# zhaihongjia/SplatLoc

Hardware: AMD Instinct MI355X
Metric: fwd+bwd frames/s @1080p, 500k Gaussians, 32 feat-ch; HBM GB/s vs roofline (higher is better)
Workload: dtype f32

## Files before the change

include/splatraster.h:

```cpp
#ifndef SPLATRASTER_H
#define SPLATRASTER_H

#include <stddef.h>
#include <stdint.h>

#ifdef __cplusplus
extern "C" {
#endif

#define SPLATRASTER_ABI_VERSION 20

#define SPLATRASTER_TILE 16

#define SPLATRASTER_OK 0
#define SPLATRASTER_ERR_BAD_ARG 1
#define SPLATRASTER_ERR_HIP 2
#define SPLATRASTER_ERR_UNSUPPORTED 3
#define SPLATRASTER_ERR_OVERFLOW 4
#define SPLATRASTER_WARN_LOOKBACK_STALL 5

typedef struct splatraster_settings {
    int32_t image_height;
    int32_t image_width;
    float tanfovx;
// ... 557 lines not shown
                               float* grad_h, uint8_t* valid, void* stream);

#define SPLATRASTER_GRAD_MASK_REPLICA 0
#define SPLATRASTER_GRAD_MASK_GLOBAL 1
int splatraster_grad_mask_workspace_bytes(int32_t N, int32_t H, int32_t W, int32_t mode, int32_t have_intensity, size_t* bytes);
int splatraster_grad_mask(int32_t N, int32_t H, int32_t W, const float* images, float edge_threshold, float eps, int32_t mode,
                          int32_t out_u8, void* out, float* intensity, float* thresholds, void* workspace, size_t workspace_bytes,
                          void* stream);
int splatraster_debug_image_ops_path(int32_t H, int32_t W);

int splatraster_masked_median_workspace_bytes(int32_t N, int64_t n, size_t* bytes);
int splatraster_masked_median(int32_t N, int64_t n, const float* values, int32_t positive_only, const float* opacity,
                              float opacity_min, const uint8_t* mask, float* median, float* std, int64_t* count, uint8_t* valid,
                              void* workspace, size_t workspace_bytes, void* stream);



int splatraster_sp_nms_tile(int32_t* tile_h, int32_t* tile_w);
int splatraster_sp_workspace_bytes(int32_t B, int32_t H, int32_t W, int32_t max_keypoints, size_t* bytes);
int splatraster_sp_scores(int32_t B, int32_t Hc, int32_t Wc, const float* semi, float* scores, void* stream);
int splatraster_sp_nms(int32_t B, int32_t H, int32_t W, const float* scores, int32_t radius, float* out, void* stream);
int splatraster_sp_select(int32_t B, int32_t H, int32_t W, const float* nms, float threshold, int32_t max_keypoints, int32_t border,
                          float* keypoints, float* scores, int32_t* count, int32_t* candidates, void* workspace, size_t workspace_bytes,
                          void* stream);
int splatraster_sp_sample(int32_t B, int32_t Hc, int32_t Wc, const float* coarse, int32_t K, const float* keypoints, const int32_t* count,
                          float* descriptors, void* workspace, size_t workspace_bytes, void* stream);
int splatraster_sp_dense_descriptors(int32_t B, int32_t Hc, int32_t Wc, const float* coarse, int32_t row0, int32_t rows, float* out,
                                     void* workspace, size_t workspace_bytes, void* stream);


int splatraster_poll_errors(void);
int splatraster_debug_set_spin_limit(uint32_t limit);
int splatraster_debug_set_deterministic(int on);
int splatraster_debug_set_small_panel_max_waves(int waves);
int splatraster_debug_set_split_max_waves(int waves);
int splatraster_debug_set_fwd_team(int mode);
int splatraster_debug_set_payload_stream_min(int64_t instances);
int splatraster_debug_set_payload_compact(int mode);
int splatraster_debug_set_dead_marks(int on);
int splatraster_debug_set_front_end(int mode);
int splatraster_debug_set_tile_sort_cap(int keys);
int splatraster_debug_set_sort_fork(int mode);
int splatraster_debug_exp2(int64_t n, const float* x, float* y, void* stream);
int splatraster_debug_poison_lds(uint32_t pattern, void* stream);

const char* splatraster_error_string(int status);
const char* splatraster_last_hip_error(void);
int splatraster_abi_version(void);

#ifdef __cplusplus
}
#endif
#endif
```

splatloc_amd/_native.py:

```python
from __future__ import annotations

import ctypes as C
import os

from . import build as _build

_LIB = None
ABI_VERSION = 20
ERR_UNSUPPORTED = 3

OK = 0
WARN_LOOKBACK_STALL = 5
_ERR_NAMES = {1: "bad argument", 2: "HIP runtime error", 3: "unsupported configuration",
              4: "tile instance count overflow", 5: "look-back stall (results late, never wrong)"}


class Settings(C.Structure):
    _fields_ = [
        ("image_height", C.c_int32),
        ("image_width", C.c_int32),
        ("tanfovx", C.c_float),
        ("tanfovy", C.c_float),
        ("scale_modifier", C.c_float),
        ("sh_degree", C.c_int32),
# ... 213 lines not shown
    "splatraster_densify_workspace_bytes": (_sz, [_i32]),
    "splatraster_densify_plan": (C.c_int, [C.POINTER(Model), _vp, _vp, C.c_float, C.c_float, C.c_float, C.c_float, _i32,
                                           _i32, _vp, C.POINTER(_i32), _vp]),
    "splatraster_densify_plan_thresholds": (C.c_int, [C.POINTER(Model), _vp, _vp, C.c_float, C.c_float, C.c_float,
                                                      C.c_float, _i32, _i32, _vp, C.POINTER(_i32), _vp]),
    "splatraster_densify_apply": (C.c_int, [C.POINTER(Model), C.POINTER(Model), C.POINTER(Model), _vp, C.c_uint64,
                                            C.c_uint64, _vp, _i32, C.POINTER(Model), C.POINTER(Model), C.POINTER(Model),
                                            _vp, _vp, _vp]),
    "splatraster_model_append": (C.c_int, [C.POINTER(Model)] * 7 + [_vp]),
    "splatraster_adam_step": (C.c_int, [_i32, C.POINTER(AdamGroup), C.c_double, C.c_double, C.c_double, C.c_float, _vp]),
    "splatraster_adam_step_radii": (C.c_int, [_i32, C.POINTER(AdamGroup), C.c_double, C.c_double, C.c_double, C.c_float, _i32, _vp, _vp, _vp]),
    "splatraster_adam_step_gated": (C.c_int, [_i32, C.POINTER(AdamGroup), C.c_double, C.c_double, C.c_double, C.c_float, _vp, _vp]),
    "splatraster_adam_step_radii_gated": (C.c_int, [_i32, C.POINTER(AdamGroup), C.c_double, C.c_double, C.c_double, C.c_float, _i32, _vp,
                                                    _vp, _vp, _vp]),
    "splatraster_isotropic_loss_workspace_bytes": (_sz, [_i32]),
    "splatraster_isotropic_loss": (C.c_int, [_i32, _i32, _vp, _vp, _vp, _vp, _vp, _vp]),
    "splatraster_mapping_loss_workspace_bytes": (_sz, [_i32]),
    "splatraster_mapping_loss": (C.c_int, [_i32] + [_vp] * 6 + [C.c_float] + [_vp] * 7),
    "splatraster_mapping_loss_window": (C.c_int, [_i32, _i32, _vp, C.c_float, _vp, _vp, _vp]),
    "splatraster_refinement_loss_workspace_bytes": (_sz, [_i32, _i32, _i32]),
    "splatraster_refinement_loss": (C.c_int, [_i32, _i32, _i32, C.c_float] + [_vp] * 6),
    "splatraster_eval_metrics_workspace_bytes": (_sz, [_i32, _i32, _i32]),
    "splatraster_eval_metrics": (C.c_int, [_i32, _i32, _i32] + [_vp] * 5),
    "splatraster_l1_rgbd_loss": (C.c_int, [_i64, _vp, _vp, _i64, _vp, _vp, C.c_float, _vp, _vp, _vp, _vp]),
    "splatraster_pose_step": (C.c_int, [_vp] * 5 + [C.c_float] * 5 + [C.c_int] + [_vp] * 5),
    "splatraster_l1_rgbd_loss_window": (C.c_int, [_i32, C.POINTER(L1View), _i64, _i64, C.c_float, _vp, _vp]),
    "splatraster_pose_step_window": (C.c_int, [_i32] + [_vp] * 5 + [C.c_float] * 5 + [C.c_int] + [_vp] * 5),
    "splatraster_error_string": (C.c_char_p, [C.c_int]),
    "splatraster_last_hip_error": (C.c_char_p, []),
    "splatraster_abi_version": (C.c_int, []),
    "splatraster_poll_errors": (C.c_int, []),
    "splatraster_debug_set_spin_limit": (C.c_int, [C.c_uint32]),
    "splatraster_debug_set_deterministic": (C.c_int, [C.c_int]),
    "splatraster_debug_exp2": (C.c_int, [_i64, _vp, _vp, _vp]),
    "splatraster_debug_poison_lds": (C.c_int, [C.c_uint32, _vp]),
}


def lib_path() -> str:
    return _build.LIB_PATH


def load(build_if_missing: bool = True):
    global _LIB
    if _LIB is not None:
        return _LIB
    path = os.environ.get("SPLATRASTER_LIB", _build.LIB_PATH)
    if path == _build.LIB_PATH and build_if_missing and _build.have_hipcc():
        try:
            _build.build()
        except Exception as e:
            raise RuntimeError(
                "splatloc_amd: the HIP extension libsplatraster.so could not be built "
                f"({e}). There is no CPU fallback.") from e
    if not os.path.exists(path):
        raise RuntimeError(f"{path} is missing and hipcc is not available: run `python -m splatloc_amd.build` "
                           "on a machine with ROCm. There is no CPU fallback.")
    lib = C.CDLL(path)
    lib.splatraster_abi_version.restype = C.c_int
    got = int(lib.splatraster_abi_version())
    if got != ABI_VERSION:
        raise RuntimeError(f"{path} has ABI version {got}, this binding needs {ABI_VERSION}: stale library, "
                           "rebuild with `python -m splatloc_amd.build --force`")
    for name, (res, args) in SYMBOLS.items():
        fn = getattr(lib, name)
        fn.restype = res
# ... 81 lines not shown
```

splatloc_amd/csrc/capi.hip:

```cpp
#include <assert.h>
#include <string.h>

#include <mutex>
#include <unordered_map>
#include <string>
#include <vector>

#include "common.h"

namespace sr {

static thread_local std::string g_last_error;
static int g_deterministic = 0;
static int g_split_max_waves = SPLIT_MAX_WAVES;
static int g_fwd_team = -1;
static int g_payload_compact = -1;
static int g_dead_marks = 1;
static int g_bin_mode = -1;

void set_hip_error(hipError_t e, const char* what)
{
    g_last_error = std::string(what) + ": " + hipGetErrorString(e);
}

// ... 1000 lines not shown
    return SPLATRASTER_OK;
}

int splatraster_debug_set_split_max_waves(int waves)
{
    g_split_max_waves = waves < 0 ? SPLIT_MAX_WAVES : (waves > SPLIT_MAX_WAVES ? SPLIT_MAX_WAVES : waves);
    return SPLATRASTER_OK;
}

int splatraster_debug_set_fwd_team(int mode)
{
    g_fwd_team = mode < 0 ? -1 : (mode > 2 ? 2 : mode);
    return SPLATRASTER_OK;
}

int splatraster_mark_visible(int32_t P, const float* means3D, const float* viewmatrix,
                             const float* projmatrix, uint8_t* present, void* stream)
{
    (void)projmatrix;
    if (P < 0) return SPLATRASTER_ERR_BAD_ARG;
    if (P == 0) return SPLATRASTER_OK;
    if (!means3D || !viewmatrix || !present) return SPLATRASTER_ERR_BAD_ARG;
    return launch_mark_visible(P, means3D, viewmatrix, present, reinterpret_cast<hipStream_t>(stream));
}

int splatraster_poll_errors(void) { return lookback_error_poll(); }

int splatraster_debug_set_deterministic(int on)
{
    g_deterministic = on ? 1 : 0;
    return SPLATRASTER_OK;
}

int splatraster_debug_set_spin_limit(uint32_t limit)
{
    int st = lookback_error_init();
    if (st) return st;
    return lookback_set_spin_limit(limit);
}

int splatraster_debug_exp2(int64_t n, const float* x, float* y, void* stream)
{
    if (n < 0) return SPLATRASTER_ERR_BAD_ARG;
    if (n == 0) return SPLATRASTER_OK;
    if (!x || !y) return SPLATRASTER_ERR_BAD_ARG;
    return launch_debug_exp2(n, x, y, reinterpret_cast<hipStream_t>(stream));
}

int splatraster_debug_poison_lds(uint32_t pattern, void* stream)
{
    return launch_poison_lds(pattern, reinterpret_cast<hipStream_t>(stream));
}

size_t splatraster_sort_tmp_bytes(int64_t n)
{
    const size_t m = (size_t)(n > 0 ? n : 1);
    return align_up(4 * m, 256) * 2 + sort_tmp_bytes(n);
}

static int sort_in_place(bool keys16, int64_t n, uint32_t* keys, uint32_t* vals, int32_t key_bits, void* tmp, void* stream_)
{
    if (!keys || !vals || !tmp) return SPLATRASTER_ERR_BAD_ARG;
    {
        int st0 = lookback_error_init();
        if (st0) return st0;
    }
// ... 91 lines not shown
```

splatloc_amd/csrc/common.h:

```cpp
#pragma once
#include <hip/hip_runtime.h>
#include <stdint.h>

#include "../../include/splatraster.h"

namespace sr {

constexpr int TILE = SPLATRASTER_TILE;
constexpr int TILE_PIX = TILE * TILE;
constexpr float NEAR_Z = 0.2f;
constexpr float DILATION = 0.3f;
constexpr float ALPHA_MAX = 0.99f;
constexpr float ALPHA_MIN = 1.0f / 255.0f;
constexpr float T_EPS = 0.0001f;
constexpr int WAVE = 64;
constexpr int PREPROCESS_BLOCK = 256;
static inline int preprocess_blocks(int32_t P) { return (P + PREPROCESS_BLOCK - 1) / PREPROCESS_BLOCK; }

void set_hip_error(hipError_t e, const char* what);
void set_error_text(const char* text);

int lookback_error_init();
int lookback_error_poll();
int lookback_set_spin_limit(uint32_t limit);
// ... 207 lines not shown
    uint32_t capacity;
    uint32_t tag;
    uint32_t* status;
    uint32_t* mirror;
};
struct BoundedStatus {
    uint32_t* dev;
    uint32_t* host;
    uint32_t* host_dev;
    int device;
};
int launch_bounded_status_clear(const BoundedStatus& st, hipStream_t stream);
int launch_bin_scatter_sort(const FramePlan& p, const GeomView& g, const uint32_t* table, const BinView& b, uint64_t* keys,
                            hipStream_t stream, const BoundedRun* bd = nullptr);

int launch_emit(const FramePlan& p, int64_t R, const GeomView& g, uint32_t* keys, uint32_t* vals, uint32_t* ranges,
                uint32_t nranges, hipStream_t stream, bool keys16 = false );
int launch_ranges_clear(int32_t tiles, uint32_t* ranges, hipStream_t stream);
int launch_payload(const FramePlan& p, int64_t R, const GeomView& g, const BinView& b, hipStream_t stream);
int launch_payload_compact(const FramePlan& p, int64_t R, const GeomView& g, const BinView& b, uint32_t* cranges, hipStream_t stream);
int launch_pad_features(int32_t P, int C, const float* feat, float* featp, hipStream_t stream);
static inline int padded_channels(int C) { return (C + 3) & ~3; }
constexpr int POSE_SETS = 16, POSE_SET_FLOATS = 64;
constexpr size_t POSE_ACC_BYTES = (size_t)POSE_SETS * POSE_SET_FLOATS * sizeof(float) + 256;
constexpr int POSE_ACC_FLOATS = (int)(POSE_ACC_BYTES / sizeof(float));
__host__ __device__ constexpr int gacc_moment_offset(int C) { return ((C & 15) + 7 <= 16) ? C : ((C + 15) & ~15); }
__host__ __device__ constexpr int gacc_row_floats(int C) { return (gacc_moment_offset(C) + 7 + 15) & ~15; }
__host__ __device__ constexpr int gacc_shared_floats(int C) { return C >= 32 ? (C & ~15) : 0; }
__host__ __device__ constexpr int gacc_view_floats(int C) { return gacc_row_floats(C) - gacc_shared_floats(C); }
__host__ __device__ static inline size_t gacc_total_floats(int C, size_t P, size_t V)
{
    return P * (size_t)gacc_shared_floats(C) + V * P * (size_t)gacc_view_floats(C);
}
struct GaccLayout {
    uint32_t SH, PV;
    uint32_t P;
    __host__ __device__ size_t index(size_t g, size_t i, uint32_t col) const
    {
        return col < SH ? i * SH + col : (size_t)P * SH + g * PV + (col - SH);
    }
    __host__ __device__ uint32_t view_base24(uint32_t row0) const { return P * SH + row0 * PV - SH; }
    __host__ __device__ uint32_t stride24(uint32_t col) const { return col < SH ? SH : PV; }
    __host__ __device__ uint32_t base24(uint32_t col, uint32_t row0) const { return col < SH ? 0u : view_base24(row0); }
};
__host__ __device__ constexpr int gacc_det_headroom_drop(int C, int V) { return (gacc_shared_floats(C) > 0 && V > 1) ? 3 : 0; }
__host__ __device__ static inline GaccLayout gacc_layout(int C, int32_t P)
{
    return GaccLayout{(uint32_t)gacc_shared_floats(C), (uint32_t)gacc_view_floats(C), (uint32_t)P};
}
#ifndef SR_SPLIT_MAX_WAVES
#define SR_SPLIT_MAX_WAVES 6144
#endif
constexpr int SPLIT_MAX_WAVES = SR_SPLIT_MAX_WAVES;
constexpr int SPLIT_MIN_LIST = 256;
#ifndef SR_SPLIT_PARTS
#define SR_SPLIT_PARTS 4
#endif
constexpr int SPLIT_PARTS = SR_SPLIT_PARTS;
constexpr int SPLIT_PARTS_MAX = 4 * SPLIT_PARTS;
#ifndef SR_SPLIT_LONG
#define SR_SPLIT_LONG 1024
#endif
#ifndef SR_SPLIT_EXTRA_TILES
#define SR_SPLIT_EXTRA_TILES 512
#endif
constexpr int SPLIT_LONG = SR_SPLIT_LONG, SPLIT_EXTRA_TILES = SR_SPLIT_EXTRA_TILES;
// ... 31 lines not shown
```

splatloc_amd/csrc/composite_bwd.hip:

```cpp
#include <type_traits>

#include "composite_common.h"

#ifndef SR_BWD_FS
#define SR_BWD_FS 32
#endif
#ifndef SR_BWD_STAGE_UNROLL
#define SR_BWD_STAGE_UNROLL 3
#endif

#ifndef SR_BWD_MINW
#define SR_BWD_MINW 4
#endif

#ifndef SR_BWD_DOT_CHAINS
#define SR_BWD_DOT_CHAINS 2
#endif
#ifndef SR_BWD_SMALL_PANEL_MAX_WAVES
#define SR_BWD_SMALL_PANEL_MAX_WAVES 6144
#endif
#ifndef SR_BWD_DOT_PREFETCH
#define SR_BWD_DOT_PREFETCH 1
#endif
#ifndef SR_BWD_TM
// ... 33 lines not shown
{
    const int eb = (int)((max_bits >> 23) & 0xffu);
    return DET_HEADROOM_EXP - (eb > 0 ? eb : 1);
}
template <bool DET>
__device__ __forceinline__ void acc_add(float* gacc, long long* gacc64, size_t idx, float v, int det_pass, int det_drop)
{
    if (DET) {
        if (det_pass == 0) {
            atomicMax(reinterpret_cast<unsigned*>(gacc) + idx, __float_as_uint(fabsf(v)));
        } else {
            const unsigned mb = __builtin_nontemporal_load(reinterpret_cast<const unsigned*>(gacc) + idx);
            if (((mb >> 23) & 0xffu) == 0xffu) {
                if (__builtin_isinf(v)) atomicAdd(reinterpret_cast<unsigned long long*>(gacc64) + idx, v > 0.f ? 1ull : (1ull << 32));
                return;
            }
            const double scaled = ldexp((double)v, det_scale_exp(mb) - det_drop);
            atomicAdd(reinterpret_cast<unsigned long long*>(gacc64) + idx, (unsigned long long)__double2ll_rn(scaled));
        }
    } else {
        (void)det_pass;
        (void)det_drop;
        atomicAdd(gacc + idx, v);
    }
}

__device__ __forceinline__ float walk_divide(float T, float one_minus_alpha) { return T * __builtin_amdgcn_rcpf(one_minus_alpha); }
__device__ __forceinline__ double walk_divide(double T, double one_minus_alpha) { return T / one_minus_alpha; }
__device__ __forceinline__ float walk_fma(float a, float b, float c) { return fmaf(a, b, c); }
__device__ __forceinline__ double walk_fma(double a, double b, double c) { return fma(a, b, c); }
template <typename ST>
__device__ __forceinline__ void walk_entry(ST& T, ST& A, bool hit, float alpha, float q, float& dA, float& w)
{
    const ST Ti = hit ? walk_divide(T, (ST)1 - (ST)alpha) : T;
    const ST d = (ST)q - A;
    dA = (float)(Ti * d);
    const ST ah = hit ? (ST)alpha : (ST)0;
    A = walk_fma(ah, d, A);
    w = (float)(ah * Ti);
    T = Ti;
}

enum class GaccTable { SHARED, VIEW, BY_COLUMN };
template <bool DET>
struct GradRows {
    float* __restrict__ gacc;
    long long* __restrict__ gacc64;
    GaccLayout GL;
    uint32_t row0, pv_base;
    int det_pass, det_drop;
    __device__ __forceinline__ uint32_t stride(uint32_t col, GaccTable tb) const
    {
        return tb == GaccTable::SHARED ? GL.SH : (tb == GaccTable::VIEW ? GL.PV : GL.stride24(col));
    }
    __device__ __forceinline__ uint32_t offset(uint32_t col, GaccTable tb) const
    {
        return (tb == GaccTable::SHARED ? 0u : (tb == GaccTable::VIEW ? pv_base : GL.base24(col, row0))) + col;
    }
    static __device__ __forceinline__ size_t index(uint32_t id, uint32_t stride, uint32_t offset) { return (size_t)(__umul24(id, stride) + offset); }
    __device__ __forceinline__ size_t index(uint32_t id, uint32_t col, GaccTable tb) const { return index(id, stride(col, tb), offset(col, tb)); }
    __device__ __forceinline__ void add(size_t idx, float v) const { acc_add<DET>(gacc, gacc64, idx, v, det_pass, det_drop); }
};

template <int NC, bool SP, bool AUX>
constexpr int bwd_min_waves() { return (BwdCfg<NC, SP, AUX>::TM && NC >= 32) ? SR_BWD_MINW_TM : SR_BWD_MINW; }

template <int NC, bool DET, bool SP, bool AUX>
__global__ void __launch_bounds__(WAVE, (bwd_min_waves<NC, SP, AUX>()))
composite_bwd_kernel(int W, int H, int C_total, int CP4, int c0, int first_pass, int tiles , int V,
                     int P ,
                     const uint32_t* __restrict__ ranges, const uint32_t* __restrict__ ipack ,
                     const float4* __restrict__ irec, const float4* __restrict__ featp4,
                     WinGrad grads,
                     const float* __restrict__ final_T_all, const uint32_t* __restrict__ n_contrib_all,
                     float* __restrict__ gacc , GaccLayout GL,
                     int MO , long long* __restrict__ gacc64 ,
                     const float* __restrict__ ckpt_all ,
                     const uint32_t* __restrict__ nparts ,
                     int extra_blocks ,
                     const uint32_t* __restrict__ tile_order ,
                     int det_pass ,
                     uint32_t cand_bits )
{
    using Cfg = BwdCfg<NC, SP, AUX>;
    using ST = typename std::conditional<DET, double, float>::type;
    constexpr int NCP = Cfg::NCP, NM = Cfg::NM, NV = Cfg::NV, KV = Cfg::KV, FS = Cfg::FS;
    constexpr int WS = Cfg::WS, GROUP = Cfg::GROUP;
    constexpr bool MFMA = Cfg::MFMA, XD = Cfg::XD;
    constexpr int NB = Cfg::NB;
    constexpr bool TM = Cfg::TM;
    constexpr int EG = Cfg::EG, ES = Cfg::ES;
    constexpr bool DOTM = NC >= SR_BWD_DOTM_MIN;
    constexpr int PPR = NCP / 4;
    static_assert(2 * KV <= WAVE, "at most 25 butterfly-reduced channels per pass");
    __shared__ __attribute__((aligned(16))) float4 s_rec0[FS + 1];
    __shared__ __attribute__((aligned(16))) float4 s_rec1[FS + 1];
    __shared__ __attribute__((aligned(16))) float s_feat[(FS + (DOTM ? 0 : 1)) * NCP];
    __shared__ uint32_t s_cgid[FS + 1];
    __shared__ float s_w[MFMA ? WAVE * WS : 1];
    __shared__ uint32_t s_gid[MFMA ? GROUP : 1];
    __shared__ float s_e[TM ? WAVE * ES : 1];
    __shared__ float2 s_emean[TM ? GROUP : 1];

    int gtile, quad;
    const int gx = tile_columns(W);
    int seg_y = (int)blockIdx.y;
    if (NC <= 4 && (int)blockIdx.x < extra_blocks) {
        const unsigned per = quadrant_blocks(SPLIT_EXTRA_TILES, gx);
        const unsigned group = blockIdx.x / per;
        int r;
        quadrant_of_block(blockIdx.x - group * per, SPLIT_EXTRA_TILES, gx, r, quad);
        if (r >= SPLIT_EXTRA_TILES || r >= V * tiles) return;
        gtile = (int)tile_order[r];
        seg_y += SPLIT_PARTS * (int)(group + 1u);
        if (seg_y >= (int)nparts[gtile]) return;
    } else {
        quadrant_of_block(blockIdx.x - (NC <= 4 ? (unsigned)extra_blocks : 0u), V * tiles, gx, gtile, quad, tile_order);
        if (gtile >= V * tiles) return;
    }
    const int lane = threadIdx.x;
    const QuadFrame F = quadrant_frame(W, H, tiles, V, P, ranges, gtile, quad, lane);
    const int view = F.view;
    const uint32_t row0 = F.row0;
    const bool inside = F.inside;
    const size_t plane = F.plane, pix = F.pix;
    constexpr bool WIDE = NC >= 32;
    const int det_drop = DET ? gacc_det_headroom_drop(C_total, V) : 0;
    static_assert(!WIDE || (Cfg::NM == 32 && NC < 48), "a wide kernel's flush columns are the shared table's, its butterfly columns the per-view row's");
    constexpr bool FIXED = NC == 35;
    static_assert(!FIXED || (gacc_shared_floats(NC) == 32 && gacc_view_floats(NC) == 16 && gacc_shared_floats(NC + 1) == 32 &&
                             gacc_view_floats(NC + 1) == 16), "the constants of the headline kernel");
    if constexpr (FIXED) { GL.SH = 32u; GL.PV = 16u; }
    const GradRows<DET> rows{gacc, gacc64, GL, row0, GL.view_base24(row0), det_pass, det_drop};
    constexpr GaccTable FLUSH_COLS = WIDE ? GaccTable::SHARED : GaccTable::BY_COLUMN, BUTTERFLY_COLS = WIDE ? GaccTable::VIEW : GaccTable::BY_COLUMN;
    const float* __restrict__ dL_dcolor = grads.dL_dcolor[view];
    const float* __restrict__ dL_ddepth = grads.dL_ddepth[view];
    const float* __restrict__ dL_dalpha = grads.dL_dalpha[view];
    const float* __restrict__ dL_dlast = grads.dL_dlast[view];
    const int gc = grads.gc;
    const float* __restrict__ final_T = final_T_all + (size_t)view * H * W;
    const uint32_t* __restrict__ n_contrib = n_contrib_all + (size_t)view * H * W;
    const float fx = (float)F.px, fy = (float)F.py;
    uint32_t beg = F.beg, end0 = F.end;
    const uint32_t list0 = beg;
    const bool split = !DET && NC <= 4 && ckpt_all != nullptr;
    const int seg = split ? seg_y : 0;
    const SplitParts parts = split_parts(split, nparts, gtile, end0 - beg);
    const int np = parts.np;
    if (split) {
        take_part(parts, seg, beg, end0);
        if (beg >= end0) return;
    }
    uint32_t last = inside ? n_contrib[pix] : 0u;
    uint32_t wave_last = last;
#pragma unroll
    for (int d = 1; d < WAVE; d <<= 1) wave_last = max(wave_last, (uint32_t)__shfl_xor((int)wave_last, d, WAVE));
    uint32_t end = min(end0, list0 + wave_last);
    if constexpr (WIDE) end = (uint32_t)__builtin_amdgcn_readfirstlane((int)end);
    if (beg >= end) return;
    float g[NC];
    ST A = 0;
    ST T = 1;
    float gD = 0.0f;
    if (inside) {
        const bool from_ckpt = split && seg < np - 1 && list0 + last > end0;
        float s_end = 0.0f;
// ... 58 lines not shown
                }
                const float Tb = *segment_record(ckpt_all, F, C_total, seg + 1, 0);
                T = (ST)Tb;
                A = (ST)(sfx / Tb);
            }
        }
    } else {
#pragma unroll
        for (int ch = 0; ch < NC; ++ch) g[ch] = 0.0f;
    }
    float gt[MFMA ? 16 : 1][NB];
    if (MFMA) {
#pragma unroll
        for (int t = 0; t < NB; ++t) {
            __builtin_amdgcn_wave_barrier();
#pragma unroll
            for (int ch = 0; ch < 16; ++ch) {
                const int c = 16 * t + ch;
                s_w[lane * WS + ch] = c < NC ? g[c < NC ? c : 0] : ((XD && c == NC) ? gD : 0.0f);
            }
            __builtin_amdgcn_wave_barrier();
#pragma unroll
            for (int kk = 0; kk < 16; ++kk) gt[kk][t] = s_w[(4 * kk + (lane >> 4)) * WS + (lane & 15)];
        }
        __builtin_amdgcn_wave_barrier();
    }

    const int slotv = (int)(__brev((unsigned)lane) >> 26);
    const bool slot_second = slotv >= KV;
    const int sv = slot_second ? slotv - KV : slotv;
    const bool slot_col = sv < NV;
    const bool slot_ok = slotv < 2 * KV;
    const uint32_t slot_colv = (uint32_t)(slot_col ? (c0 + NM + sv) : (TM ? MO + 6 : MO + sv - NV));
    const uint32_t slot_stride = rows.stride(slot_colv, BUTTERFLY_COLS), slot_off = rows.offset(slot_colv, BUTTERFLY_COLS);
    int nslot = 0;
    int e0 = 0;

    auto flush_panel = [&](int count) {
        __builtin_amdgcn_wave_barrier();
        f32x4 D[NB];
#pragma unroll
        for (int t = 0; t < NB; ++t) D[t] = f32x4{0.f, 0.f, 0.f, 0.f};
        const int row = (lane >> 4) * WS + (lane & 15);
#pragma unroll
        for (int kk = 0; kk < 16; ++kk) {
            const float a = s_w[4 * kk * WS + row];
#pragma unroll
            for (int t = 0; t < NB; ++t) {
                D[t] = __builtin_amdgcn_mfma_f32_16x16x4f32(a, gt[kk][t], D[t], 0, 0, 0);
            }
        }
        const int j0c = lane & 15;
#pragma unroll
        for (int r = 0; r < 4; ++r) {
            const int gs = 4 * (lane >> 4) + r;
            if (gs < count) {
                const uint32_t gid = s_gid[gs];
#pragma unroll
                for (int t = 0; t < NB; ++t) {
                    const int c = 16 * t + j0c;
                    const bool full = 16 * t + 16 <= NM;
                    const bool col_ok = full || c < NM || (XD && c == NM && first_pass);
                    const uint32_t col = (full || c < NM) ? (uint32_t)(c0 + c) : (uint32_t)(MO + 6);
                    if (col_ok) rows.add(rows.index(gid, col, FLUSH_COLS), D[t][r]);
                }
            }
        }
        __builtin_amdgcn_wave_barrier();
    };

    auto reduce_e = [&](int count) {
        if constexpr (TM) {
            __builtin_amdgcn_wave_barrier();
            const int eg = lane & 7, ei = lane >> 3;
            const float2 mu = s_emean[min(e0 + eg, GROUP - 1)];
            const float dx = mu.x - (float)(F.qx + ei);
            const float dy0 = mu.y - (float)F.qy;
            float m[6] = {0.f, 0.f, 0.f, 0.f, 0.f, 0.f};
#pragma unroll
            for (int j = 0; j < 8; ++j) {
                const float e = s_e[(8 * j + ei) * ES + eg];
                const float dy = dy0 - (float)j;
                const float ey = e * dy;
                m[5] += e;
                m[1] += ey;
// ... 10 lines not shown
            __builtin_amdgcn_wave_barrier();
        }
    };

    uint32_t pw = 0;
    auto fetch = [&](uint32_t base, uint32_t& w_) {
        w_ = 0u;
        if (base + (uint32_t)lane < end) w_ = ipack[base + (uint32_t)lane];
    };
    const uint64_t gt_mask = (lane == WAVE - 1) ? 0ull : (~0ull << (lane + 1));
    const int nchunks = (int)((end - beg + (WAVE - 1)) / WAVE);
    fetch(beg + (uint32_t)(nchunks - 1) * WAVE, pw);

#pragma unroll 1
    for (int chunk = nchunks - 1; chunk >= 0; --chunk) {
        const uint32_t base = beg + (uint32_t)chunk * WAVE;
        const bool cur_reach = (pw & (cand_bits << quad)) == (IPACK_REACH0 << quad);
        uint64_t cand = __builtin_amdgcn_ballot_w64(cur_reach);
        const uint32_t cur_gid = (pw & 0xFFFFFFu) - row0;
        fetch(chunk > 0 ? base - WAVE : 0xFFFFFF00u, pw);
        const uint32_t idx0 = base - list0;
#pragma unroll 1
        while (cand != 0) {
            const int ncand = min(FS, (int)__popcll(cand));
            const int rank = __popcll(cand & gt_mask);
            const bool mine = cur_reach && ((cand >> lane) & 1ull) && rank < FS;
            __builtin_amdgcn_wave_barrier();
            if (mine) s_cgid[rank] = cur_gid;
            float4 rec_a = make_float4(0.f, 0.f, 0.f, 0.f), rec_b = rec_a;
            if (mine) {
                const size_t j = (size_t)base + lane;
                rec_a = irec[2 * j];
                rec_b = irec[2 * j + 1];
            }
            __builtin_amdgcn_wave_barrier();
#pragma unroll SR_BWD_STAGE_UNROLL
            for (int e = lane; e < ncand * PPR; e += WAVE) {
                const int row = e / PPR, pc = e - row * PPR;
                reinterpret_cast<float4*>(s_feat)[e] = featp4[(size_t)(__umul24(s_cgid[row], (uint32_t)CP4) + (uint32_t)((c0 >> 2) + pc))];
            }
            if (mine) {
                s_rec0[rank] = rec_a;
                s_rec1[rank] = rec_b;
            }
            __builtin_amdgcn_wave_barrier();
            auto process_pair = [&](int j0, int j1, bool has1, int r0, int r1, float qm0, float qm1) {
                const int r[2] = {r0, r1};
                float4 p[2], q[2];
                float dx[2], dy[2];
                for (int e = 0; e < 2; ++e) p[e] = s_rec0[r[e]], q[e] = s_rec1[r[e]];
                for (int e = 0; e < 2; ++e) dx[e] = p[e].x - fx, dy[e] = p[e].y - fy;
                const PairAlpha pa = pair_alpha(q[0], dx[0], dy[0], q[1], dx[1], dy[1]);
                const float al[2] = {pa.al0, pa.al1}, Gr[2] = {pa.G0, pa.G1};
                auto contributes = [&](int je, bool pass) { return (idx0 + (uint32_t)je < last) && pass; };
                const bool hit0 = contributes(j0, pa.pass0), hit1 = has1 && contributes(j1, pa.pass1);
                const float G[2] = {hit0 ? Gr[0] : 0.0f, hit1 ? Gr[1] : 0.0f};
                float qd[2] = {qm0, qm1};
                if (!DOTM) {
                    for (int e = 0; e < 2; ++e) qd[e] = AUX ? p[e].z * gD : 0.0f;
#pragma unroll
                    for (int ch = 0; ch < NC; ++ch) {
                        for (int e = 0; e < 2; ++e) qd[e] += s_feat[r[e] * NCP + ch] * g[ch];
                    }
                    qd[1] = has1 ? qd[1] : 0.0f;
                }
                float dA[2], w[2], E[2];
                uint32_t gi[2];
                walk_entry<ST>(T, A, hit0, al[0], qd[0], dA[0], w[0]);
                walk_entry<ST>(T, A, hit1, al[1], qd[1], dA[1], w[1]);
                for (int e = 0; e < 2; ++e) E[e] = G[e] * dA[e];
                for (int e = 0; e < 2; ++e) gi[e] = s_cgid[r[e]];
                if constexpr (KV > 0) {
                    float red[2 * KV];
#pragma unroll
                    for (int ch = 0; ch < NV; ++ch) {
                        for (int e = 0; e < 2; ++e) red[e * KV + ch] = w[e] * g[NM + ch];
                    }
                    if constexpr (!TM) {
                        for (int e = 0; e < 2; ++e) {
                            const float Ex = E[e] * dx[e], Ey = E[e] * dy[e];
                            red[e * KV + NV + 0] = Ex;
                            red[e * KV + NV + 1] = Ey;
                            red[e * KV + NV + 2] = Ex * dx[e];
                            red[e * KV + NV + 3] = Ex * dy[e];
                            red[e * KV + NV + 4] = Ey * dy[e];
                            red[e * KV + NV + 5] = E[e];
                        }
                    }
                    if constexpr (!XD && AUX) {
                        for (int e = 0; e < 2; ++e) red[e * KV + KV - 1] = w[e] * gD;
                    }
                    {
                        const float outv = wave_reduce_pack<2 * KV>(red, lane);
                        const uint32_t gid = slot_second ? gi[1] : gi[0];
                        if (slot_ok && (has1 || !slot_second)) rows.add(rows.index(gid, slot_stride, slot_off), outv);
                    }
                }
                if constexpr (MFMA) {
                    for (int e = 0; e < 2; ++e) s_w[lane * WS + nslot + e] = w[e];
                    if constexpr (TM) {
                        for (int e = 0; e < 2; ++e) s_e[lane * ES + (nslot - e0) + e] = E[e];
                    }
                    if (lane == 0) {
                        for (int e = 0; e < 2; ++e) s_gid[nslot + e] = gi[e];
                        if constexpr (TM) {
                            for (int e = 0; e < 2; ++e) s_emean[nslot + e] = make_float2(p[e].x, p[e].y);
                        }
                    }
                    nslot += has1 ? 2 : 1;
                    if constexpr (TM) {
                        if (nslot - e0 >= EG - 1 || nslot >= GROUP - 1) {
                            reduce_e(nslot - e0);
                            e0 = nslot;
                        }
                    }
                    if (nslot >= GROUP - 1) {
                        flush_panel(nslot);
                        nslot = 0;
                        e0 = 0;
                    }
                }
            };
            auto dot4 = [&](int slot4) -> f32x4 {
                const int k = lane & 3;
                const int srow = min(slot4 + k, ncand - 1);
                const float* fr = &s_feat[srow * NCP];
                const float zsel = reinterpret_cast<const float*>(&s_rec0[srow])[2];
                constexpr int CH = SR_BWD_DOT_CHAINS;
// ... 29 lines not shown
            for (int slot = 0; slot < ncand; slot += (DOTM ? 4 : 2)) {
                const bool has1 = slot + 1 < ncand, has2 = DOTM && slot + 2 < ncand, has3 = DOTM && slot + 3 < ncand;
                const int j0 = 63 - __builtin_clzll(cand);
                cand &= ~(1ull << j0);
                const int j1 = has1 ? 63 - __builtin_clzll(cand) : j0;
                if (has1) cand &= ~(1ull << j1);
                const int j2 = has2 ? 63 - __builtin_clzll(cand) : j1;
                if (has2) cand &= ~(1ull << j2);
                const int j3 = has3 ? 63 - __builtin_clzll(cand) : j2;
                if (has3) cand &= ~(1ull << j3);
                float qm[4] = {0.f, 0.f, 0.f, 0.f};
                if (DOTM) {
                    const f32x4 Q = dot4(slot);
                    qm[0] = Q[0]; qm[1] = Q[1]; qm[2] = Q[2]; qm[3] = Q[3];
                }
                process_pair(j0, j1, has1, slot, slot + 1, qm[0], qm[1]);
                if (has2) process_pair(j2, j3, has3, slot + 2, slot + 3, qm[2], qm[3]);
            }
        }
    }
    if constexpr (TM) { if (nslot - e0 > 0) reduce_e(nslot - e0); }
    if (MFMA && nslot > 0) flush_panel(nslot);
}



static int g_small_panel_max_waves = SR_BWD_SMALL_PANEL_MAX_WAVES;
void set_small_panel_max_waves(int waves) { g_small_panel_max_waves = waves < 0 ? SR_BWD_SMALL_PANEL_MAX_WAVES : waves; }

struct BwdLaunch {
    const WinGrad* grads;
    const float* ckpt;
    int det_pass;
};

template <int NC, bool DET, bool AUX = true>
static int launch_one_bwd(const FramePlan& p, int c0, int first, const BinView& b, const ImgView& im, const float* feat,
                          int feat_stride, const BwdLaunch& L, float* gacc, long long* gacc64, hipStream_t stream)
{
    const int gx = p.gx, tiles = p.tiles;
    const unsigned blocks = quadrant_blocks((int)p.gtiles, gx);
    const float* ckpt = (NC <= 4 && c0 == 0 && first) ? L.ckpt : nullptr;
    const GaccLayout GL = gacc_layout(p.C, p.P);
    if (NC == 35 && (c0 != 0 || GL.SH != 32u || GL.PV != 16u)) return SPLATRASTER_ERR_UNSUPPORTED;
    const bool extras = ckpt != nullptr && p.order;
    const unsigned extra_blocks = extras ? (unsigned)(SPLIT_PARTS_MAX / SPLIT_PARTS - 1) * quadrant_blocks(SPLIT_EXTRA_TILES, gx) : 0u;
    const dim3 grid(blocks + extra_blocks, ckpt ? (unsigned)SPLIT_PARTS : 1u);
#define SR_BWD_LAUNCH(SPV)                                                                                          \
    hipLaunchKernelGGL((composite_bwd_kernel<NC, DET, SPV, AUX>), grid, dim3(WAVE), 0, stream, p.W,                     \
                       p.H, feat_stride, padded_channels(feat_stride) / 4, c0, first, tiles, p.V, p.P,                 \
                       b.ranges, b.ipack, b.irec, reinterpret_cast<const float4*>(feat), *L.grads,       \
                       im.final_T, im.n_contrib, gacc, GL,                                                             \
                       gacc_moment_offset(p.C), gacc64, ckpt, extras ? b.nparts : nullptr, (int)extra_blocks,                      \
                       p.order ? b.tile_order : nullptr, L.det_pass, p.dead_marks ? IPACK_REACH0 | IPACK_DEAD0 : IPACK_REACH0)
    if constexpr (NC >= 4 && NC <= 15 && AUX) {
        if (4 * tiles <= g_small_panel_max_waves)
            SR_BWD_LAUNCH(true);
        else
            SR_BWD_LAUNCH(false);
    } else {
        SR_BWD_LAUNCH(false);
    }
#undef SR_BWD_LAUNCH
    SR_LAUNCH_CHECK();
    return SPLATRASTER_OK;
}

int launch_composite_bwd(const FramePlan& p, int64_t R, const BinView& b, const ImgView& im, const float* feat, int feat_stride,
                         const WinGrad& grads, float* gacc, long long* gacc64, int det_pass, hipStream_t stream)
{
    if (R == 0) return SPLATRASTER_OK;
    const bool det = gacc64 != nullptr;
    int C = p.C;
    const int V = p.V;
    const BwdLaunch L{&grads, (!det && p.split) ? b.ckpt : nullptr, det_pass};
    bool any_last = false, any_aux = false;
    for (int v = 0; v < V; ++v) {
        any_last = any_last || grads.dL_dlast[v] != nullptr;
        any_aux = any_aux || grads.dL_ddepth[v] != nullptr || grads.dL_dalpha[v] != nullptr;
    }
    if (grads.gc < C && !any_last && !det) C = grads.gc;
    if (C == 3 && !any_aux && !det)
        return launch_one_bwd<3, false, false>(p, 0, 1, b, im, feat, feat_stride, L, gacc, gacc64, stream);
#define SR_BWD_ARGS b, im, feat, feat_stride, L, gacc, gacc64, stream
#define SR_BWD_ONE(N, c0_, first_) (det ? launch_one_bwd<N, true>(p, c0_, first_, SR_BWD_ARGS) : launch_one_bwd<N, false>(p, c0_, first_, SR_BWD_ARGS))
    if (C == 35) return SR_BWD_ONE(35, 0, 1);
    int c0 = 0, first = 1, st = SPLATRASTER_OK;
    while (c0 < C && st == SPLATRASTER_OK) {
        const int left = C - c0;
        if (left >= 32) { st = SR_BWD_ONE(32, c0, first); c0 += 32; }
        else if (left >= 16) { st = SR_BWD_ONE(16, c0, first); c0 += 16; }
        else if (left >= 8) { st = SR_BWD_ONE(8, c0, first); c0 += 8; }
        else if (left >= 4) { st = SR_BWD_ONE(4, c0, first); c0 += 4; }
        else if (left == 3) { st = SR_BWD_ONE(3, c0, first); c0 += 3; }
        else if (left == 2) { st = SR_BWD_ONE(2, c0, first); c0 += 2; }
        else { st = SR_BWD_ONE(1, c0, first); c0 += 1; }
        first = 0;
    }
#undef SR_BWD_ONE
#undef SR_BWD_ARGS
    return st;
}

}
```

splatloc_amd/csrc/composite_common.h:

```cpp
#pragma once
#include <type_traits>

#include "common.h"

namespace sr {

__device__ __forceinline__ unsigned quadrant_reach_mask(const float4 r0, const float4 r1, float tile_x0,
                                                        float tile_y0)
{
    const float A = r1.x, B = r1.y, C = r1.z;
    const float lim0 = 2.0f * __logf(255.0f * r1.w);
    const float lim = lim0 + 0.02f + 1e-4f * fabsf(lim0);
    if (!(lim > 0.0f)) return 0u;
    const float nBrA = -B * __frcp_rn(A), nBrC = -B * __frcp_rn(C);
    unsigned mask = 0u;
#pragma unroll
    for (int q = 0; q < 4; ++q) {
        const float bx0 = tile_x0 + (float)((q & 1) * 8), by0 = tile_y0 + (float)((q >> 1) * 8);
        const float u0 = r0.x - (bx0 + 7.0f), u1 = r0.x - bx0;
        const float v0 = r0.y - (by0 + 7.0f), v1 = r0.y - by0;
        float qmin;
        if (u0 <= 0.0f && u1 >= 0.0f && v0 <= 0.0f && v1 >= 0.0f) {
            qmin = 0.0f;
        } else {
// ... 177 lines not shown
__device__ __forceinline__ float fold_lane_bit3(float x, float y)
{
#if !SR_BUTTERFLY_ASM
    const bool lo = (__lane_id() & 8) == 0;
    const float keep = lo ? x : y, send = lo ? y : x;
    return keep + dpp_get<0x128, 0xf>(send);
#endif
    float d;
    asm("s_nop 1\n\t"
        "v_add_f32_dpp %0, %1, %1 row_ror:8 row_mask:0xf bank_mask:0x3\n\t"
        "v_add_f32_dpp %0, %2, %2 row_ror:8 row_mask:0xf bank_mask:0xc"
        : "=&v"(d)
        : "v"(x), "v"(y));
    return d;
}
__device__ __forceinline__ float fold_lane_bit2(float x, float y)
{
#if !SR_BUTTERFLY_ASM
    const bool lo = (__lane_id() & 4) == 0;
    const float keep = lo ? x : y, send = lo ? y : x;
    float t = dpp_mov_old<0x12C, 0x5>(0.0f, send);
    t = dpp_mov_old<0x124, 0xA>(t, send);
    return keep + t;
#endif
    float d;
    asm("s_nop 1\n\t"
        "v_add_f32_dpp %0, %1, %1 row_ror:12 row_mask:0xf bank_mask:0x5\n\t"
        "v_add_f32_dpp %0, %2, %2 row_ror:4 row_mask:0xf bank_mask:0xa"
        : "=&v"(d)
        : "v"(x), "v"(y));
    return d;
}

template <int K>
__device__ __forceinline__ float wave_reduce_pack(const float (&v)[K], int lane)
{
    static_assert(K >= 1 && K <= 64, "at most 64 values per wave");
    constexpr int N1 = (K + 1) / 2, N2 = (N1 + 1) / 2, N3 = (N2 + 1) / 2, N4 = (N3 + 1) / 2,
                  N5 = (N4 + 1) / 2, N6 = (N5 + 1) / 2;
    static_assert(N6 == 1, "");
    float a[N1];
#pragma unroll
    for (int m = 0; m < N1; ++m) {
        const float x = v[2 * m];
        const float y = (2 * m + 1 < K) ? v[2 * m + 1] : 0.0f;
        const auto r = __builtin_amdgcn_permlane32_swap(as_u(x), as_u(y), false, false);
        a[m] = as_f(r[0]) + as_f(r[1]);
    }
    float b[N2];
#pragma unroll
    for (int m = 0; m < N2; ++m) {
        const float x = a[2 * m];
        const float y = (2 * m + 1 < N1) ? a[2 * m + 1] : 0.0f;
        const auto r = __builtin_amdgcn_permlane16_swap(as_u(x), as_u(y), false, false);
        b[m] = as_f(r[0]) + as_f(r[1]);
    }
    float c[N3];
#pragma unroll
    for (int m = 0; m < N3; ++m)
        c[m] = (2 * m + 1 < N2) ? fold_lane_bit3(b[2 * m], b[2 * m + 1 < N2 ? 2 * m + 1 : 0]) : b[2 * m] + dpp_get<0x128, 0xf>(b[2 * m]);
    float d[N4];
#pragma unroll
    for (int m = 0; m < N4; ++m)
        d[m] = (2 * m + 1 < N3) ? fold_lane_bit2(c[2 * m], c[2 * m + 1 < N3 ? 2 * m + 1 : 0]) : fold_lane_bit2(c[2 * m], c[2 * m]);
    float e[N5];
    {
        const bool lo = (lane & 2) == 0;
#pragma unroll
        for (int m = 0; m < N5; ++m) {
            const float x = d[2 * m];
            if (2 * m + 1 < N4) {
                const float y = d[2 * m + 1 < N4 ? 2 * m + 1 : 0];
                const float keep = lo ? x : y, send = lo ? y : x;
                e[m] = keep + dpp_get<0x4E, 0xf>(send);
            } else {
                e[m] = x + dpp_get<0x4E, 0xf>(x);
            }
        }
    }
    const float x6 = e[0];
    if (N5 > 1) {
        const bool lo1 = (lane & 1) == 0;
        const float y6 = e[N5 > 1 ? 1 : 0];
        const float keep6 = lo1 ? x6 : y6, send6 = lo1 ? y6 : x6;
        return keep6 + dpp_get<0xB1, 0xf>(send6);
    }
    return x6 + dpp_get<0xB1, 0xf>(x6);
}

template <int K>
__device__ __forceinline__ float wave_reduce_hi3(const float (&v)[K], int lane)
{
    static_assert(K >= 1 && K <= 8, "at most 8 values");
    constexpr int N1 = (K + 1) / 2, N2 = (N1 + 1) / 2;
    float a[N1];
#pragma unroll
    for (int m = 0; m < N1; ++m) {
        const float x = v[2 * m];
        const float y = (2 * m + 1 < K) ? v[2 * m + 1] : 0.0f;
        const auto r = __builtin_amdgcn_permlane32_swap(as_u(x), as_u(y), false, false);
        a[m] = as_f(r[0]) + as_f(r[1]);
    }
    float b[N2];
#pragma unroll
    for (int m = 0; m < N2; ++m) {
        const float x = a[2 * m];
        const float y = (2 * m + 1 < N1) ? a[2 * m + 1] : 0.0f;
        const auto r = __builtin_amdgcn_permlane16_swap(as_u(x), as_u(y), false, false);
        b[m] = as_f(r[0]) + as_f(r[1]);
    }
    (void)lane;
    if (N2 > 1) return fold_lane_bit3(b[0], b[N2 > 1 ? 1 : 0]);
    return b[0] + dpp_get<0x128, 0xf>(b[0]);
}

}
```

Measured before the change: 762.8.

## Use 32-bit byte offsets for gradient atomics and carry gaussian id in record

In the fixed headline backward kernel, gradient accumulator atomics switch to 32-bit byte offsets when the whole accumulator fits under 4 GiB, so 64-bit index arithmetic is avoided. The gaussian id is stored in the unused w component of the per-instance record instead of being looked up from an LDS table. The walk_entry select is reordered into a branch-free form, and the final DPP fold uses inline asm. A debug query for the short-offset predicate is exposed; the new path adds template variants and depends on the size check staying correct.

```diff
diff --git a/include/splatraster.h b/include/splatraster.h
--- a/include/splatraster.h
+++ b/include/splatraster.h
@@ -613,6 +613,7 @@
 int splatraster_poll_errors(void);
 int splatraster_debug_set_spin_limit(uint32_t limit);
 int splatraster_debug_set_deterministic(int on);
+int splatraster_debug_gacc_short_offsets(int32_t C, int32_t P, int32_t n_views);
 int splatraster_debug_set_small_panel_max_waves(int waves);
 int splatraster_debug_set_split_max_waves(int waves);
 int splatraster_debug_set_fwd_team(int mode);
diff --git a/splatloc_amd/_native.py b/splatloc_amd/_native.py
--- a/splatloc_amd/_native.py
+++ b/splatloc_amd/_native.py
@@ -269,6 +269,7 @@
     "splatraster_poll_errors": (C.c_int, []),
     "splatraster_debug_set_spin_limit": (C.c_int, [C.c_uint32]),
     "splatraster_debug_set_deterministic": (C.c_int, [C.c_int]),
+    "splatraster_debug_gacc_short_offsets": (C.c_int, [_i32, _i32, _i32]),
     "splatraster_debug_exp2": (C.c_int, [_i64, _vp, _vp, _vp]),
     "splatraster_debug_poison_lds": (C.c_int, [C.c_uint32, _vp]),
 }
diff --git a/splatloc_amd/csrc/capi.hip b/splatloc_amd/csrc/capi.hip
--- a/splatloc_amd/csrc/capi.hip
+++ b/splatloc_amd/csrc/capi.hip
@@ -1056,6 +1056,12 @@
     return SPLATRASTER_OK;
 }
 
+int splatraster_debug_gacc_short_offsets(int32_t C, int32_t P, int32_t n_views)
+{
+    if (C <= 0 || P < 0 || n_views <= 0) return 0;
+    return gacc_short_offsets(C, (size_t)P, (size_t)n_views) ? 1 : 0;
+}
+
 int splatraster_debug_set_spin_limit(uint32_t limit)
 {
     int st = lookback_error_init();
diff --git a/splatloc_amd/csrc/common.h b/splatloc_amd/csrc/common.h
--- a/splatloc_amd/csrc/common.h
+++ b/splatloc_amd/csrc/common.h
@@ -263,6 +263,10 @@
 {
     return P * (size_t)gacc_shared_floats(C) + V * P * (size_t)gacc_view_floats(C);
 }
+__host__ __device__ static inline bool gacc_short_offsets(int C, size_t P, size_t V)
+{
+    return (unsigned long long)gacc_total_floats(C, P, V) * sizeof(float) < (1ull << 32);
+}
 struct GaccLayout {
     uint32_t SH, PV;
     uint32_t P;
diff --git a/splatloc_amd/csrc/composite_bwd.hip b/splatloc_amd/csrc/composite_bwd.hip
--- a/splatloc_amd/csrc/composite_bwd.hip
+++ b/splatloc_amd/csrc/composite_bwd.hip
@@ -89,10 +89,10 @@
 template <typename ST>
 __device__ __forceinline__ void walk_entry(ST& T, ST& A, bool hit, float alpha, float q, float& dA, float& w)
 {
-    const ST Ti = hit ? walk_divide(T, (ST)1 - (ST)alpha) : T;
+    const ST ah = hit ? (ST)alpha : (ST)0;
+    const ST Ti = walk_divide(T, (ST)1 - ah);
     const ST d = (ST)q - A;
     dA = (float)(Ti * d);
-    const ST ah = hit ? (ST)alpha : (ST)0;
     A = walk_fma(ah, d, A);
     w = (float)(ah * Ti);
     T = Ti;
@@ -106,6 +106,7 @@
     GaccLayout GL;
     uint32_t row0, pv_base;
     int det_pass, det_drop;
+    bool short_off;
     __device__ __forceinline__ uint32_t stride(uint32_t col, GaccTable tb) const
     {
         return tb == GaccTable::SHARED ? GL.SH : (tb == GaccTable::VIEW ? GL.PV : GL.stride24(col));
@@ -113,6 +114,21 @@
     __device__ __forceinline__ uint32_t offset(uint32_t col, GaccTable tb) const
     {
         return (tb == GaccTable::SHARED ? 0u : (tb == GaccTable::VIEW ? pv_base : GL.base24(col, row0))) + col;
+    }
+    __device__ __forceinline__ uint32_t units(uint32_t offset_floats) const { return short_off ? offset_floats << 2 : offset_floats; }
+    __device__ __forceinline__ void add_short(uint32_t bytes, uint32_t more, float v) const
+    {
+        atomicAdd(reinterpret_cast<float*>(reinterpret_cast<char*>(gacc) + (size_t)bytes) + more, v);
+    }
+    template <bool SHORT, uint32_t STRIDE>
+    __device__ __forceinline__ void add_fixed(uint32_t id, uint32_t off, uint32_t more, float v) const
+    {
+        if constexpr (SHORT && !DET) {
+            add_short(id * (STRIDE * 4u) + off, more, v);
+        } else {
+            add((size_t)(id * STRIDE + off) + more, v);
+            if constexpr (!DET) asm volatile("");
+        }
     }
     static __device__ __forceinline__ size_t index(uint32_t id, uint32_t stride, uint32_t offset) { return (size_t)(__umul24(id, stride) + offset); }
     __device__ __forceinline__ size_t index(uint32_t id, uint32_t col, GaccTable tb) const { return index(id, stride(col, tb), offset(col, tb)); }
@@ -137,7 +153,8 @@
                      int extra_blocks ,
                      const uint32_t* __restrict__ tile_order ,
                      int det_pass ,
-                     uint32_t cand_bits )
+                     uint32_t cand_bits ,
+                     int short_off )
 {
     using Cfg = BwdCfg<NC, SP, AUX>;
     using ST = typename std::conditional<DET, double, float>::type;
@@ -188,7 +205,7 @@
     static_assert(!FIXED || (gacc_shared_floats(NC) == 32 && gacc_view_floats(NC) == 16 && gacc_shared_floats(NC + 1) == 32 &&
                              gacc_view_floats(NC + 1) == 16), "the constants of the headline kernel");
     if constexpr (FIXED) { GL.SH = 32u; GL.PV = 16u; }
-    const GradRows<DET> rows{gacc, gacc64, GL, row0, GL.view_base24(row0), det_pass, det_drop};
+    const GradRows<DET> rows{gacc, gacc64, GL, row0, GL.view_base24(row0), det_pass, det_drop, FIXED && !DET && short_off != 0};
     constexpr GaccTable FLUSH_COLS = WIDE ? GaccTable::SHARED : GaccTable::BY_COLUMN, BUTTERFLY_COLS = WIDE ? GaccTable::VIEW : GaccTable::BY_COLUMN;
     const float* __restrict__ dL_dcolor = grads.dL_dcolor[view];
     const float* __restrict__ dL_ddepth = grads.dL_ddepth[view];
@@ -313,7 +330,8 @@
     const bool slot_col = sv < NV;
     const bool slot_ok = slotv < 2 * KV;
     const uint32_t slot_colv = (uint32_t)(slot_col ? (c0 + NM + sv) : (TM ? MO + 6 : MO + sv - NV));
-    const uint32_t slot_stride = rows.stride(slot_colv, BUTTERFLY_COLS), slot_off = rows.offset(slot_colv, BUTTERFLY_COLS);
+    const uint32_t slot_stride = rows.stride(slot_colv, BUTTERFLY_COLS);
+    const uint32_t slot_off = FIXED ? rows.units(rows.offset(slot_colv, BUTTERFLY_COLS)) : rows.offset(slot_colv, BUTTERFLY_COLS);
     int nslot = 0;
     int e0 = 0;
 
@@ -332,6 +350,24 @@
             }
         }
         const int j0c = lane & 15;
+        if constexpr (FIXED) {
+            const uint32_t off = rows.units((uint32_t)j0c);
+            auto add_rows = [&](auto form) {
+#pragma unroll
+                for (int r = 0; r < 4; ++r) {
+                    const int gs = 4 * (lane >> 4) + r;
+                    if (gs < count) {
+                        const uint32_t gid = s_gid[gs];
+#pragma unroll
+                        for (int t = 0; t < NB; ++t) rows.template add_fixed<decltype(form)::value, 32u>(gid, off, 16u * (uint32_t)t, D[t][r]);
+                    }
+                }
+            };
+            if (rows.short_off) add_rows(std::true_type{});
+            else add_rows(std::false_type{});
+            __builtin_amdgcn_wave_barrier();
+            return;
+        }
 #pragma unroll
         for (int r = 0; r < 4; ++r) {
             const int gs = 4 * (lane >> 4) + r;
@@ -408,6 +444,7 @@
                 const size_t j = (size_t)base + lane;
                 rec_a = irec[2 * j];
                 rec_b = irec[2 * j + 1];
+                if constexpr (FIXED) rec_a.w = __uint_as_float(cur_gid);
             }
             __builtin_amdgcn_wave_barrier();
 #pragma unroll SR_BWD_STAGE_UNROLL
@@ -445,7 +482,7 @@
                 walk_entry<ST>(T, A, hit0, al[0], qd[0], dA[0], w[0]);
                 walk_entry<ST>(T, A, hit1, al[1], qd[1], dA[1], w[1]);
                 for (int e = 0; e < 2; ++e) E[e] = G[e] * dA[e];
-                for (int e = 0; e < 2; ++e) gi[e] = s_cgid[r[e]];
+                for (int e = 0; e < 2; ++e) gi[e] = FIXED ? __float_as_uint(p[e].w) : s_cgid[r[e]];
                 if constexpr (KV > 0) {
                     float red[2 * KV];
 #pragma unroll
@@ -469,7 +506,14 @@
                     {
                         const float outv = wave_reduce_pack<2 * KV>(red, lane);
                         const uint32_t gid = slot_second ? gi[1] : gi[0];
-                        if (slot_ok && (has1 || !slot_second)) rows.add(rows.index(gid, slot_stride, slot_off), outv);
+                        if (slot_ok && (has1 || !slot_second)) {
+                            if constexpr (FIXED) {
+                                if (rows.short_off) rows.template add_fixed<true, 16u>(gid, slot_off, 0u, outv);
+                                else rows.template add_fixed<false, 16u>(gid, slot_off, 0u, outv);
+                            } else {
+                                rows.add(rows.index(gid, slot_stride, slot_off), outv);
+                            }
+                        }
                     }
                 }
                 if constexpr (MFMA) {
@@ -565,6 +609,7 @@
     const WinGrad* grads;
     const float* ckpt;
     int det_pass;
+    bool short_off;
 };
 
 template <int NC, bool DET, bool AUX = true>
@@ -585,7 +630,8 @@
                        b.ranges, b.ipack, b.irec, reinterpret_cast<const float4*>(feat), *L.grads,       \
                        im.final_T, im.n_contrib, gacc, GL,                                                             \
                        gacc_moment_offset(p.C), gacc64, ckpt, extras ? b.nparts : nullptr, (int)extra_blocks,                      \
-                       p.order ? b.tile_order : nullptr, L.det_pass, p.dead_marks ? IPACK_REACH0 | IPACK_DEAD0 : IPACK_REACH0)
+                       p.order ? b.tile_order : nullptr, L.det_pass, p.dead_marks ? IPACK_REACH0 | IPACK_DEAD0 : IPACK_REACH0,  \
+                       (int)L.short_off)
     if constexpr (NC >= 4 && NC <= 15 && AUX) {
         if (4 * tiles <= g_small_panel_max_waves)
             SR_BWD_LAUNCH(true);
@@ -606,7 +652,7 @@
     const bool det = gacc64 != nullptr;
     int C = p.C;
     const int V = p.V;
-    const BwdLaunch L{&grads, (!det && p.split) ? b.ckpt : nullptr, det_pass};
+    const BwdLaunch L{&grads, (!det && p.split) ? b.ckpt : nullptr, det_pass, gacc_short_offsets(p.C, (size_t)p.P, (size_t)p.V)};
     bool any_last = false, any_aux = false;
     for (int v = 0; v < V; ++v) {
         any_last = any_last || grads.dL_dlast[v] != nullptr;
diff --git a/splatloc_amd/csrc/composite_common.h b/splatloc_amd/csrc/composite_common.h
--- a/splatloc_amd/csrc/composite_common.h
+++ b/splatloc_amd/csrc/composite_common.h
@@ -233,6 +233,19 @@
     return d;
 }
 
+__device__ __forceinline__ float fold_lane_bit0(float x)
+{
+#if !SR_BUTTERFLY_ASM
+    return x + dpp_get<0xB1, 0xf>(x);
+#endif
+    float d;
+    asm("s_nop 1\n\t"
+        "v_add_f32_dpp %0, %1, %1 quad_perm:[1,0,3,2] row_mask:0xf bank_mask:0xf"
+        : "=v"(d)
+        : "v"(x));
+    return d;
+}
+
 template <int K>
 __device__ __forceinline__ float wave_reduce_pack(const float (&v)[K], int lane)
 {
@@ -286,7 +299,7 @@
         const float keep6 = lo1 ? x6 : y6, send6 = lo1 ? y6 : x6;
         return keep6 + dpp_get<0xB1, 0xf>(send6);
     }
-    return x6 + dpp_get<0xB1, 0xf>(x6);
+    return fold_lane_bit0(x6);
 }
 
 template <int K>
```

After: 770.8 (median of 6 runs). 1.01x the previous value.
